# nianticlabs/mickey

Hardware: AMD Instinct MI355X
Metric: image pairs/sec (540x720) (higher is better)
Workload: dtype bf16

## Files before the change

### mickey_amd/csrc/mk_gemm_common.hpp

```cpp
#pragma once
#include "mk_common.hpp"

namespace mk {
namespace gemm {

constexpr int BK = 64;
template <typename T> constexpr int EPC = 16 / (int)sizeof(T);
template <typename T> constexpr int KT = 128 / (int)sizeof(T);

enum AMode { A_DENSE = 0, A_CONV3 = 1 };

struct GemmParams {
  const void* A;
  const void* A2;
  const void* W;
  int M, N, K, lda, ldw;
  long long strideA_g, strideA2_g, strideW_g;
  int H, Wd, C1, C2;
  int bord_out;
  unsigned pl1[2], pl2[2];
  int npass;
  float acc_scale;
  void* out_lo;
  float plane_scale;
// ... 496 lines not shown
  const int fr = lane & 15, fg = lane >> 4;
  const float* bias = HAS_BIAS ? p.bias + (long long)g * p.strideBias_g : nullptr;
  const int nw = n0 + wn * 64;
  const int mw = m0 + wm * 128;
  int img0 = 0, tok0 = 0;
  if (EPI == MK_EPI_QKV) {
    img0 = mw / p.ntok;
    tok0 = mw - img0 * p.ntok;
  }
  auto img_tok = [&](int r, int& img, int& tok) {
    if (p.ntok >= 128) {
      const int t = tok0 + r;
      const bool wrap = t >= p.ntok;
      img = img0 + (wrap ? 1 : 0);
      tok = wrap ? t - p.ntok : t;
    } else {
      const int m = mw + r;
      img = m / p.ntok;
      tok = m - img * p.ntok;
    }
  };
  f32x4 bv[4], cs[4];
#pragma unroll
  for (int ni = 0; ni < 4; ++ni) {
    const int n = nw + fg * 4 + ni * 16;
    bv[ni] = (HAS_BIAS && n < p.N) ? *(const f32x4*)(bias + n) : f32x4{0.f, 0.f, 0.f, 0.f};
    cs[ni] = (LN && n < p.N) ? *(const f32x4*)(p.ln_colsum + n) : f32x4{0.f, 0.f, 0.f, 0.f};
  }
  float2 prm[8];
#pragma unroll
  for (int mi = 0; mi < 8; ++mi) prm[mi] = LN ? lnp[wm * 128 + mi * 16 + fr] : make_float2(1.f, 0.f);
  const bool lp_out = EPI == MK_EPI_QKV || (EPI == MK_EPI_STORE && !p.out_f32 && !p.out_lo);
  if (lp_out) {
    int which = 0, head = 0;
    if (EPI == MK_EPI_QKV) {
      const int D = p.heads * 64;
      which = nw / D;
      head = (nw - which * D) >> 6;
      if (which == 2) {
#pragma unroll
        for (int mi = 0; mi < 8; ++mi) {
          const int m = mw + mi * 16 + fr;
          if (m >= p.M) continue;
          int img, tok;
          img_tok(mi * 16 + fr, img, tok);
          const long long hb = (long long)img * p.heads + head;
#pragma unroll
          for (int ni = 0; ni < 4; ++ni) {
            const f32x4 v = LN ? acc[mi][ni] * prm[mi].x + (cs[ni] * prm[mi].y + bv[ni]) : acc[mi][ni] + bv[ni];
            T* dst = (T*)p.vt + (hb * 64 + ni * 16 + fg * 4) * p.ntok_pad + vperm(tok);
#pragma unroll
            for (int e = 0; e < 4; ++e) dst[(long long)e * p.ntok_pad] = to_lp<T>(v[e]);
          }
        }
        return;
      }
    }
    const int rr = lane >> 3, c = lane & 7;
    const int n = nw + c * 8;
    const bool bord = CONV && p.bord_out;
    BorderedRow bw;
    if (bord) bw.init(mw + rr, p.H, p.Wd);
#pragma unroll
    for (int h = 0; h < 2; ++h) {
#pragma unroll
      for (int mq = 0; mq < 4; ++mq) {
        const int mi = h * 4 + mq;
        const int r = mi * 16 + fr;
        char* wrow = (mq < 2 ? wl0 : wl1) + ((mq & 1) * 16 + fr) * 128;
        const long long rrow = (CONV && p.resid_lp) ? bordered_row(min(mw + r, p.M - 1), p.H, p.Wd) : 0;
#pragma unroll
        for (int ni = 0; ni < 4; ++ni) {
          f32x4 v = acc[mi][ni];
          if (LN) v = v * prm[mi].x + (cs[ni] * prm[mi].y + bv[ni]);
          else if (HAS_BIAS) v += bv[ni];
          if (EPI == MK_EPI_QKV) {
            if (which == 0) { const float qs = p.qscale; _Pragma("unroll") for (int e = 0; e < 4; ++e) v[e] *= qs; }
          } else {
            if (CONV && p.resid_lp) {
              const int m = mw + r, n2 = nw + fg * 4 + ni * 16;
              if (m < p.M && n2 < p.N) {
                const V4 rs = *(const V4*)((const T*)p.resid_lp + (long long)g * p.strideResid_g + rrow * p.ldc + n2);
#pragma unroll
                for (int e = 0; e < 4; ++e) v[e] += (float)rs[e];
              }
            }
            if (ACT == MK_ACT_RELU) {
#pragma unroll
              for (int e = 0; e < 4; ++e) v[e] = fmaxf(v[e], 0.f);
            } else if (ACT == MK_ACT_GELU) {
              v = gelu_erf4(v);
            }
          }
          V4 o;
#pragma unroll
          for (int e = 0; e < 4; ++e) o[e] = to_lp<T>(v[e]);
          const int cc = ni * 2 + (fg >> 1);
          *(V4*)(wrow + ((cc ^ (fr & 7)) << 4) + (fg & 1) * 8) = o;
        }
      }
#pragma unroll
      for (int i8 = 0; i8 < 8; ++i8) {
        const int it = h * 8 + i8;
        const int r = it * 8 + rr;
        const int m = mw + r;
        const V8 val = *(const V8*)((i8 < 4 ? wl0 : wl1) + ((i8 & 3) * 8 + rr) * 128 + ((c ^ (rr & 7)) << 4));
        const int extra = bord ? bw.extra : 0;
        if (bord) bw.step(8, p.H, p.Wd);
        if (m >= p.M || n >= p.N) continue;
        T* dst;
        if (EPI == MK_EPI_QKV) {
          int img, tok;
          img_tok(r, img, tok);
          dst = (T*)(which == 0 ? p.q : p.k) + (((long long)img * p.heads + head) * p.ntok_pad + tok) * 64 + c * 8;
        } else {
          dst = (T*)p.out_lp + (long long)g * p.strideOut_g + ((long long)m + extra) * p.ldc + n;
        }
        if (n + 8 <= p.N) {
          *(V8*)dst = val;
        } else {
          V4 lo;
#pragma unroll
          for (int e = 0; e < 4; ++e) lo[e] = val[e];
          *(V4*)dst = lo;
        }
      }
    }
  } else {
    const int rr = lane >> 4, c = lane & 15;
    const int n = nw + c * 4;
    f32x4 gm = f32x4{0.f, 0.f, 0.f, 0.f};
    if (EPI == MK_EPI_LS_RESIDUAL && n < p.N) gm = *(const f32x4*)(p.gamma + n);
    f32x4 bvd = f32x4{0.f, 0.f, 0.f, 0.f};
    if (SPLIT && HAS_BIAS && n < p.N) bvd = *(const f32x4*)(bias + n);
    f32x4 xr[2][SPLIT ? 1 : 16];
    uint2 xh[2][SPLIT ? 16 : 1], xl[2][SPLIT ? 16 : 1];
    const unsigned lane_off = (unsigned)rr * (unsigned)p.ldxs + (unsigned)n;
    unsigned lane_off_st = lane_off;
    asm volatile("" : "+v"(lane_off_st));
    auto plane_row = [&](void* plane, int half, int it) -> T* {
      return (T*)plane + (long long)(mw + half * 64 + it * 4) * p.ldxs;
    };
    __amdgpu_buffer_rsrc_t rs_h, rs_l;
    unsigned voff_b = 0;
    if constexpr (SPLIT && EPI == MK_EPI_LS_RESIDUAL && sizeof(T) == 2) {
      rs_h = __builtin_amdgcn_make_buffer_rsrc(p.xh, 0, 0x7fffffff, 0x00020000);
      rs_l = __builtin_amdgcn_make_buffer_rsrc(p.xl, 0, 0x7fffffff, 0x00020000);
      voff_b = lane_off * 2u;
    }
    auto soff_b = [&](int half, int it) -> unsigned {
      return (unsigned)(mw + half * 64 + it * 4) * (unsigned)p.ldxs * 2u;
    };
    typedef unsigned u32x2_t __attribute__((ext_vector_type(2)));
    auto preload = [&](int half, int it0 = 0, int it1 = 16) {
      if (EPI != MK_EPI_LS_RESIDUAL) return;
#pragma unroll
      for (int it = 0; it < 16; ++it) {
        if (it < it0 || it >= it1) continue;
        const int m = mw + half * 64 + it * 4 + rr;
        const bool ok = SPLIT || (m < p.M && n < p.N);
        if constexpr (SPLIT && EPI == MK_EPI_LS_RESIDUAL && sizeof(T) == 2) {
          const u32x2_t a = __builtin_amdgcn_raw_buffer_load_b64(rs_h, voff_b, soff_b(half, it), 0);
          const u32x2_t b = __builtin_amdgcn_raw_buffer_load_b64(rs_l, voff_b, soff_b(half, it), 0);
          xh[half][it] = uint2{a[0], a[1]};
          xl[half][it] = uint2{b[0], b[1]};
        } else if (SPLIT) {
          xh[half][it] = ok ? *(const uint2*)(plane_row(p.xh, half, it) + lane_off) : uint2{0u, 0u};
          xl[half][it] = ok ? *(const uint2*)(plane_row(p.xl, half, it) + lane_off) : uint2{0u, 0u};
        } else {
          xr[half][it] = ok ? *(const f32x4*)(p.out_f32 + (long long)m * p.ldc + n) : f32x4{0.f, 0.f, 0.f, 0.f};
        }
      }
    };
    auto stageq = [&](int half, int sub) {
#pragma unroll
      for (int m2 = 0; m2 < 2; ++m2) {
        const int mi = sub * 2 + m2;
        const int r = mi * 16 + fr;
        char* wrow = (m2 == 0 ? wl0 : wl1) + fr * 256;
        const long long rrow = (CONV && p.resid_lp) ? bordered_row(min(mw + half * 64 + r, p.M - 1), p.H, p.Wd) : 0;
#pragma unroll
        for (int ni = 0; ni < 4; ++ni) {
          f32x4 v = acc[half * 4 + mi][ni];
          if (EPI == MK_EPI_STORE && p.npass > 1) {
            const float sc = p.acc_scale;
#pragma unroll
            for (int e = 0; e < 4; ++e) v[e] *= sc;
          }
          if (HAS_BIAS && !SPLIT) v += bv[ni];
          if (EPI == MK_EPI_STORE) {
            if (CONV && p.resid_lp) {
              const int m = mw + half * 64 + r, nn = nw + fg * 4 + ni * 16;
              if (m < p.M && nn < p.N) {
                const V4 rs = *(const V4*)((const T*)p.resid_lp + (long long)g * p.strideResid_g + rrow * p.ldc + nn);
#pragma unroll
                for (int e = 0; e < 4; ++e) v[e] += (float)rs[e];
              }
            }
            if (ACT == MK_ACT_RELU) {
#pragma unroll
              for (int e = 0; e < 4; ++e) v[e] = fmaxf(v[e], 0.f);
            } else if (ACT == MK_ACT_GELU) {
              v = gelu_erf4(v);
            }
          }
          const int cw = ni * 4 + fg;
          *(f32x4*)(wrow + ((cw ^ fr) << 4)) = v;
        }
      }
    };
    constexpr bool fin = FIN;
    auto emit_row = [&](long long xrow, T* dh, T* dl, f32x4 x, bool ok, unsigned soff = 0xffffffffu) {
      float ssum = 0.f, qsum = 0.f;
      if (ok) {
        const uint2 oh = pack4<T>(x);
        const uint2 ol = pack4<T>(x - unpack4<T>(oh));
        quad_stats(x, ssum, qsum);
        if constexpr (SPLIT && EPI == MK_EPI_LS_RESIDUAL && sizeof(T) == 2) {
          __builtin_amdgcn_raw_buffer_store_b64(u32x2_t{oh.x, oh.y}, rs_h, voff_b, soff, 0);
          __builtin_amdgcn_raw_buffer_store_b64(u32x2_t{ol.x, ol.y}, rs_l, voff_b, soff, 0);
        } else {
          *(uint2*)dh = oh;
          *(uint2*)dl = ol;
        }
      }
      ssum = row16_sum(ssum);
      qsum = row16_sum(qsum);
      if (ok && c == 0) ((float2*)p.stats_out)[xrow * p.nslot_out + (nw >> 6)] = make_float2(ssum, qsum);
    };
    auto drain = [&](int half, int it0 = 0, int it1 = 16) {
      const bool bordf = CONV && p.bord_out;
      BorderedRow bwf;
      if (bordf) bwf.init(mw + half * 64 + it0 * 4 + rr, p.H, p.Wd);
#pragma unroll
      for (int it = 0; it < 16; ++it) {
        if (it < it0 || it >= it1) continue;
        const int r = it * 4 + rr;
        const int m = mw + half * 64 + r;
        const int extraf = bordf ? bwf.extra : 0;
        if (bordf) bwf.step(4, p.H, p.Wd);
        f32x4 val = *(const f32x4*)(((it & 4) ? wl1 : wl0) + ((it & 3) * 4 + rr) * 256 + ((c ^ ((it & 3) * 4 + rr)) << 4));
        if (SPLIT) val += bvd;
        const bool ok = SPLIT || (m < p.M && n < p.N);
        if (!ok) continue;
        if (EPI == MK_EPI_LS_RESIDUAL) {
          f32x4 x;
          if (SPLIT) {
            x = unpack4<T>(xh[half][it]) + unpack4<T>(xl[half][it]);
          } else {
            x = xr[half][it];
          }
          x += gm * val;
          if (SPLIT) x -= ((const float*)lnp)[wm * 128 + half * 64 + r];
          if (!SPLIT || fin) {
            if (ok) *(f32x4*)(p.out_f32 + (long long)m * p.ldc + n) = x;
          } else {
            if constexpr (sizeof(T) == 2) emit_row(m, nullptr, nullptr, x, ok, soff_b(half, it));
            else emit_row(m, plane_row(p.xh, half, it) + lane_off_st, plane_row(p.xl, half, it) + lane_off_st, x, ok);
          }
        } else if (EPI == MK_EPI_PATCH) {
          const int mc = ok ? m : 0;
          const int img = mc / p.npatch, tok = mc - img * p.npatch;
          const long long xrow = (long long)img * (p.npatch + 1) + 1 + tok;
          f32x4 x = val;
          if (ok) x += *(const f32x4*)(p.pos + (long long)(1 + tok) * p.N + n);
          if (SPLIT) emit_row(xrow, (T*)p.xh + xrow * p.ldxs + n, (T*)p.xl + xrow * p.ldxs + n, x, ok);
          else if (ok) *(f32x4*)(p.out_f32 + xrow * p.ldc + n) = x;
        } else if (EPI == MK_EPI_STORE && p.out_lo) {
          const float ps = p.plane_scale;
          f16x4 oh, ol;
#pragma unroll
          for (int e = 0; e < 4; ++e) {
            const float sv = sat16(val[e] * ps, p.sat_flag);
            oh[e] = (_Float16)sv;
            ol[e] = (_Float16)(sv - (float)oh[e]);
          }
          const long long o = (long long)g * p.strideOut_g + ((long long)m + extraf) * p.ldc + n;
          *(f16x4*)((_Float16*)p.out_lp + o) = oh;
          *(f16x4*)((_Float16*)p.out_lo + o) = ol;
        } else {
          *(f32x4*)(p.out_f32 + (long long)g * p.strideOut_g + ((long long)m + extraf) * p.ldc + n) = val;
        }
      }
    };
    if (SPLIT && !FIN && EPI == MK_EPI_LS_RESIDUAL) {
      preload(0, 0, 16);
      stageq(0, 0);
      drain(0, 0, 8);
      preload(1, 0, 8);
      stageq(0, 1);
      drain(0, 8, 16);
      preload(1, 8, 16);
      stageq(1, 0);
      drain(1, 0, 8);
      stageq(1, 1);
      drain(1, 8, 16);
    } else {
      preload(0);
      stageq(0, 0);
      drain(0, 0, 8);
      stageq(0, 1);
      preload(1);
      drain(0, 8, 16);
      stageq(1, 0);
      drain(1, 0, 8);
      stageq(1, 1);
      drain(1, 8, 16);
    }
  }
}

template <typename T, int KIND, bool CONV = false, int BN = 256>
__device__ __forceinline__ void epilogue_lds(const GemmParams& p, f32x4 (&acc)[8][4], char* wl0, char* wl1, int m0, int n0, int wm,
                                             int wn, int lane, int g, const float2* lnp = nullptr) {
  if constexpr (KIND == 2 || KIND == 3) {
    const bool interior = m0 + 256 <= p.M && n0 + BN <= p.N;
    if (KIND == 3) {
      if (interior) epilogue_lds_impl<T, MK_EPI_LS_RESIDUAL, MK_ACT_NONE, true, false, true, true>(p, acc, wl0, wl1, m0, n0, wm, wn, lane, g, lnp);
      else epilogue_impl<T, 8, MK_EPI_LS_RESIDUAL, MK_ACT_NONE, true, false, true>(p, acc, m0, n0, wm, wn, lane, g);
    } else if (p.epi == MK_EPI_PATCH) {
      if (interior) epilogue_lds_impl<T, MK_EPI_PATCH, MK_ACT_NONE, true, false, true>(p, acc, wl0, wl1, m0, n0, wm, wn, lane, g);
      else epilogue_impl<T, 8, MK_EPI_PATCH, MK_ACT_NONE, true, false, true>(p, acc, m0, n0, wm, wn, lane, g);
    } else {
      if (interior) epilogue_lds_impl<T, MK_EPI_LS_RESIDUAL, MK_ACT_NONE, true, false, true, false>(p, acc, wl0, wl1, m0, n0, wm, wn, lane, g, lnp);
      else epilogue_impl<T, 8, MK_EPI_LS_RESIDUAL, MK_ACT_NONE, true, false, true>(p, acc, m0, n0, wm, wn, lane, g);
    }
  } else if constexpr (KIND == 1) {
#if defined(MK_LN_ABL) && MK_LN_ABL == 2
    constexpr bool LNE = false;
#else
    constexpr bool LNE = true;
#endif
    if (p.epi == MK_EPI_QKV) epilogue_lds_impl<T, MK_EPI_QKV, MK_ACT_NONE, true, LNE>(p, acc, wl0, wl1, m0, n0, wm, wn, lane, g, lnp);
    else if (p.act == MK_ACT_GELU) epilogue_lds_impl<T, MK_EPI_STORE, MK_ACT_GELU, true, LNE>(p, acc, wl0, wl1, m0, n0, wm, wn, lane, g, lnp);
    else epilogue_lds_impl<T, MK_EPI_STORE, MK_ACT_NONE, true, LNE>(p, acc, wl0, wl1, m0, n0, wm, wn, lane, g, lnp);
  } else {
    switch (CONV ? MK_EPI_STORE : p.epi) {
      case MK_EPI_LS_RESIDUAL: epilogue_lds_impl<T, MK_EPI_LS_RESIDUAL, MK_ACT_NONE, true>(p, acc, wl0, wl1, m0, n0, wm, wn, lane, g); break;
      case MK_EPI_QKV: epilogue_lds_impl<T, MK_EPI_QKV, MK_ACT_NONE, true>(p, acc, wl0, wl1, m0, n0, wm, wn, lane, g); break;
      case MK_EPI_PATCH: epilogue_lds_impl<T, MK_EPI_PATCH, MK_ACT_NONE, true>(p, acc, wl0, wl1, m0, n0, wm, wn, lane, g); break;
      default:
        if (!p.bias) {
          if (p.act == MK_ACT_RELU) epilogue_lds_impl<T, MK_EPI_STORE, MK_ACT_RELU, false, false, false, false, CONV>(p, acc, wl0, wl1, m0, n0, wm, wn, lane, g);
          else if (!CONV && p.act == MK_ACT_GELU) epilogue_lds_impl<T, MK_EPI_STORE, MK_ACT_GELU, false>(p, acc, wl0, wl1, m0, n0, wm, wn, lane, g);
          else epilogue_lds_impl<T, MK_EPI_STORE, MK_ACT_NONE, false, false, false, false, CONV>(p, acc, wl0, wl1, m0, n0, wm, wn, lane, g);
        } else {
          if (p.act == MK_ACT_RELU) epilogue_lds_impl<T, MK_EPI_STORE, MK_ACT_RELU, true, false, false, false, CONV>(p, acc, wl0, wl1, m0, n0, wm, wn, lane, g);
          else if (!CONV && p.act == MK_ACT_GELU) epilogue_lds_impl<T, MK_EPI_STORE, MK_ACT_GELU, true>(p, acc, wl0, wl1, m0, n0, wm, wn, lane, g);
          else epilogue_lds_impl<T, MK_EPI_STORE, MK_ACT_NONE, true, false, false, false, CONV>(p, acc, wl0, wl1, m0, n0, wm, wn, lane, g);
        }
    }
  }
}

__device__ __forceinline__ void pp_tile_coords(int id, int ntm, int ntn, int PP_GM, int& tm, int& tn) {
  if (PP_GM < 0) {
    const int ng = -PP_GM;
    const int grp = id / (ntm * ng);
    const int rem = id - grp * (ntm * ng);
    const int gn = min(ng, ntn - grp * ng);
    tm = rem / gn;
    tn = grp * ng + rem - tm * gn;
    return;
  }
  const int band = id / (PP_GM * ntn);
  const int rem = id - band * (PP_GM * ntn);
  const int gm = min(PP_GM, ntm - band * PP_GM);
  tm = band * PP_GM + rem % gm;
  tn = rem / gm;
}

int num_cus();
extern int g_pp64_persist;
int launch_pp64(const GemmParams& p, int groups, int dtype, int amode, hipStream_t st, int band_m);
int launch_f32(const GemmParams& p, int groups, int amode, hipStream_t st);

}
}
```

### mickey_amd/csrc/mk_gemm_pp64.hip

```cpp
#include <type_traits>

#include "mk_gemm_common.hpp"

namespace mk {
namespace gemm {
int g_pp64_persist = 2;
namespace {

template <typename T, int AMODE, int KIND, bool PERSIST = false, bool SP = false, bool SP2 = false>
__global__ __launch_bounds__(512, 2) void gemm_pp64_kernel(GemmParams p, int band_m) {
  static_assert(!SP2 || SP, "SP2 is a form of the split-operand kernel");
  static_assert(!PERSIST || AMODE == A_DENSE, "the persistent tile loop is built for dense operands");
  static_assert(!SP || (KIND == 0 && !PERSIST && sizeof(T) == 2), "split operands: plain epilogues, one tile per workgroup");
  constexpr int BKA = SP ? BK / 2 : BK;
  using V8 = typename Lp<T>::V8;
  constexpr int WMF = 8, BM = 256, BN = 256;
  constexpr int A_BYTES = BM * 128, STAGE_BYTES = (BM + BN) * 128;
  constexpr int LN_STAGE_OFF = 2 * STAGE_BYTES + 256 * 8;
  extern __shared__ __attribute__((aligned(16))) char smem[];

  const int tid0 = threadIdx.x;
  const int wave = __builtin_amdgcn_readfirstlane(tid0 >> 6);
  int lane = tid0 & 63, tid = tid0;
  auto refresh_lane = [&]() {
// ... 244 lines not shown

  const bool ln = KIND == 1 && p.ln_stats != nullptr;
#if defined(MK_LN_ABL) && MK_LN_ABL == 1
  const bool ln_fast = false && ln;
#define MK_LN_NO_SLOW 1
#else
  const bool ln_fast = ln && p.ln_nslot == 16;
#endif
  LnRowLoads16 lnl;
  if (ln_fast) lnl.issue(p, m0, tid);
  constexpr bool PRODUCER = AMODE == A_DENSE && (KIND == 2 || KIND == 3);
  ShiftLoad shl;
  if constexpr (PRODUCER) shl.issue(p, m0, tid, 256);
  dma_a(0);
  dma_w(0);
  if constexpr (!PERSIST) dma_a(1);
  constexpr int YOUNGER = PERSIST ? 8 : 12;
  const bool publish = ln && p.ln_shift_out != nullptr && n0 == 0;
  if (ln_fast) lnl.template finish<YOUNGER>(p, tid, (float2*)(smem + 2 * STAGE_BYTES), m0, publish);
#ifndef MK_LN_NO_SLOW
  else if (ln) ln_params_to_lds<256, 512>(p, m0, tid, (float2*)(smem + 2 * STAGE_BYTES), publish);
#endif
  if constexpr (PRODUCER) shl.template finish<YOUNGER>(tid, 256, (float*)(smem + 2 * STAGE_BYTES));
  if constexpr (!PERSIST) asm volatile("s_waitcnt vmcnt(4)" ::: "memory");
  const int bstep = PERSIST ? (int)gridDim.x : 0;
  for (;;) {
    const int nbid = bid + bstep;
    const bool has_next = PERSIST && nbid < ntiles;
    int m1 = m0, n1 = n0;
    if (PERSIST && has_next) tile_origin(nbid, m1, n1);
    if constexpr (PERSIST) {
      refresh_lane();
      derive_lane();
      set_aoff(m0);
      set_woff(n0);
      dma_a(1);
      if (bid == (int)blockIdx.x) asm volatile("s_waitcnt vmcnt(4)" ::: "memory");
    }
    bool ln_pending = false;
    auto first_stage_done = [&]() {
      if constexpr (PERSIST) {
        if (ln_pending) {
          const bool publish1 = ln && p.ln_shift_out != nullptr && n0 == 0;
          if (ln_fast) {
            LnRowDma16::finish<0>(p, wave, lane, (float2*)(smem + 2 * STAGE_BYTES), smem + LN_STAGE_OFF, m0, publish1);
            asm volatile("s_waitcnt lgkmcnt(0)" ::: "memory");
            LnRowDma16::issue<2>(p, m0, wave, lane, smem + LN_STAGE_OFF);
          }
          if constexpr (PRODUCER) shl.template finish<-1>(tid, 256, (float*)(smem + 2 * STAGE_BYTES));
        }
      }
    };
    auto second_stage_done = [&]() {
      if constexpr (PERSIST) {
        if (ln_pending && ln_fast)
          LnRowDma16::finish<2>(p, wave, lane, (float2*)(smem + 2 * STAGE_BYTES), smem + LN_STAGE_OFF, m0,
                                ln && p.ln_shift_out != nullptr && n0 == 0);
      }
    };
    ln_pending = PERSIST && bid != (int)blockIdx.x;
    int kt0 = 0;
    if (wm == 0) {
      if constexpr (PERSIST) {
        stage0(0, Yes{}, Yes{}, 1, 2, Yes{});
        first_stage_done();
        stage0(1, Yes{}, Yes{}, 2, 3, No{});
        second_stage_done();
        kt0 = 2;
      }
      for (int kt = kt0; kt < nk - 2; ++kt) stage0(kt, Yes{}, Yes{}, kt + 1, kt + 2, No{});
      if constexpr (PERSIST) {
        set_aoff(m1);
        stage0(nk - 2, Yes{}, Yes{}, nk - 1, 0, No{});
        set_woff(n1);
        stage0(nk - 1, Yes{}, No{}, 0, 0, No{});
      } else {
        stage0(nk - 2, Yes{}, No{}, nk - 1, 0, No{});
        stage0(nk - 1, No{}, No{}, 0, 0, No{});
      }
      bar();
    } else {
      bar();
      if constexpr (PERSIST) {
        stage1(0, Yes{}, Yes{}, 1, 2, Yes{});
        first_stage_done();
        stage1(1, Yes{}, Yes{}, 2, 3, No{});
        second_stage_done();
        kt0 = 2;
      }
      for (int kt = kt0; kt < nk - 2; ++kt) stage1(kt, Yes{}, Yes{}, kt + 1, kt + 2, No{});
      if constexpr (PERSIST) {
        set_aoff(m1);
        stage1(nk - 2, Yes{}, Yes{}, nk - 1, 0, No{});
        set_woff(n1);
        stage1(nk - 1, Yes{}, No{}, 0, 0, No{});
      } else {
        stage1(nk - 2, Yes{}, No{}, nk - 1, 0, No{});
        stage1(nk - 1, No{}, No{}, 0, 0, No{});
      }
    }
    char* wl0 = smem + STAGE_BYTES + wave * 4096;
    refresh_lane();
    epilogue_lds<T, KIND, AMODE == A_CONV3>(p, acc, wl0, wl0 + A_BYTES, m0, n0, wm, wn, lane, g, (const float2*)(smem + 2 * STAGE_BYTES));
    if (!(PERSIST && has_next)) break;
    bid = nbid;
    m0 = m1;
    n0 = n1;
    asm volatile("" : "+s"(m0), "+s"(n0));
    refresh_lane();
    if (ln_fast) LnRowDma16::issue<0>(p, m0, wave, lane, smem + LN_STAGE_OFF);
    if constexpr (PRODUCER) shl.issue(p, m0, tid, 256);
  }
}

template <typename T, int AMODE, int KIND, bool PERSIST, bool SP = false, bool SP2 = false>
int launch_k2(const GemmParams& p, int groups, hipStream_t st, int band_m, int grid) {
  constexpr int LDS = 2 * 512 * 128 + 256 * 8 + (PERSIST && KIND == 1 ? 16384 : 0);
  static bool attr_done = false;
  if (!attr_done) {
    hipError_t e = hipFuncSetAttribute((const void*)gemm_pp64_kernel<T, AMODE, KIND, PERSIST, SP, SP2>, hipFuncAttributeMaxDynamicSharedMemorySize, LDS);
    if (e != hipSuccess) {
      mk_set_error("gemm: cannot reserve %d B of LDS: %s", LDS, hipGetErrorString(e));
      return MK_ERR_LAUNCH;
    }
    attr_done = true;
  }
  hipLaunchKernelGGL((gemm_pp64_kernel<T, AMODE, KIND, PERSIST, SP, SP2>), dim3(grid, groups, 1), dim3(512), LDS, st, p, band_m);
  MK_CHECK_LAUNCH();
  return MK_OK;
}

template <typename T, int AMODE, int KIND>
int launch_k(const GemmParams& p, int groups, hipStream_t st, int band_m) {
  const int ntm = (p.M + 255) / 256, ntn = (p.N + 255) / 256;
  if (band_m == 0) band_m = (AMODE == A_DENSE && ntn <= 4) ? -4 : 8;
  if constexpr (KIND == 0 && sizeof(T) == 2 && std::is_same<T, _Float16>::value) {
    if (p.npass == 2) {
      if constexpr (AMODE == A_CONV3) return launch_k2<T, AMODE, 0, false, true, true>(p, groups, st, band_m, ntm * ntn);
    }
    if (p.npass > 1) return launch_k2<T, AMODE, 0, false, true>(p, groups, st, band_m, ntm * ntn);
  }
  if constexpr (AMODE == A_DENSE && KIND != 0) {
    const int nk = p.K / BK, grid = num_cus() & ~7;
    const bool ok = groups == 1 && p.npass <= 1 && (nk & 1) == 0 && nk >= 4 && grid >= 8 && ntm * ntn > grid &&
                    !(KIND == 1 && p.ln_stats && p.ln_nslot != 16);
    if (g_pp64_persist != 1 && ok && !(g_pp64_persist == 2 && KIND == 1)) return launch_k2<T, AMODE, KIND, true>(p, groups, st, band_m, grid);
  }
  return launch_k2<T, AMODE, KIND, false>(p, groups, st, band_m, ntm * ntn);
}

template <typename T>
int launch_dense(const GemmParams& p, int groups, hipStream_t st, int band_m) {
  if (p.xh && p.epi == MK_EPI_LS_RESIDUAL && p.out_f32) return launch_k<T, A_DENSE, 3>(p, groups, st, band_m);
  if (p.xh) return launch_k<T, A_DENSE, 2>(p, groups, st, band_m);
  if (p.ln_stats) return launch_k<T, A_DENSE, 1>(p, groups, st, band_m);
  return launch_k<T, A_DENSE, 0>(p, groups, st, band_m);
}

}

int launch_pp64(const GemmParams& p, int groups, int dtype, int amode, hipStream_t st, int band_m) {
  if (amode == A_DENSE) return dtype == MK_BF16 ? launch_dense<__bf16>(p, groups, st, band_m) : launch_dense<_Float16>(p, groups, st, band_m);
  return dtype == MK_BF16 ? launch_k<__bf16, A_CONV3, 0>(p, groups, st, band_m) : launch_k<_Float16, A_CONV3, 0>(p, groups, st, band_m);
}

}
}
```

### mickey_amd/csrc/mk_norm.hip

```cpp
#include "mk_common.hpp"
#include "mk_gemm_common.hpp"

#include <stdarg.h>
#include <stdio.h>

namespace {
using namespace mk;

__device__ __forceinline__ void store_planes(void* hi, void* lo, long long o, const f32x4& y, float scale, int* sat_flag) {
  f16x4 oh, ol;
#pragma unroll
  for (int e = 0; e < 4; ++e) {
    const float sv = sat16(y[e] * scale, sat_flag);
    oh[e] = (_Float16)sv;
    ol[e] = (_Float16)(sv - (float)oh[e]);
  }
  *(f16x4*)((_Float16*)hi + o) = oh;
  if (lo) *(f16x4*)((_Float16*)lo + o) = ol;
}

constexpr int LN_MAXV = 8;

constexpr int LN_RPW = 4;

// ... 138 lines not shown
    if (r < rows_out && cok) {
      const long long rin = (long long)(r / rpo) * rows_per_img + skip + (r % rpo);
      v[t] = __builtin_nontemporal_load((const f32x4*)(x + rin * ldx + c));
    }
  }
#pragma unroll
  for (int t = 0; t < LNN_TRIPS; ++t) {
    const int r = r0 + 2 * t + half;
    const bool ok = r < rows_out && cok;
    float mean, rstd;
    f32x4 d;
    ln_narrow_stats(v[t], cok, D, eps, mean, rstd, d);
    if (!ok) continue;
    const long long wo = wgroup_rows > 0 ? (long long)(r / wgroup_rows) * D : 0;
    const f32x4 ww = *(const f32x4*)(w + wo + c), bb = *(const f32x4*)(b + wo + c);
    f32x4 y;
#pragma unroll
    for (int e = 0; e < 4; ++e) y[e] = ln_scale(d[e], rstd, ww[e], bb[e]);
    if (resid) {
      float* rp = resid + (long long)r * ldr + c;
      y += *(const f32x4*)rp;
      *(f32x4*)rp = y;
    }
    if (out) {
      long long ro = r;
      if (bord_h > 0) {
        const int gb = r / bord_m, m = r - gb * bord_m;
        ro = gb * bordered_rows(bord_m / (bord_h * bord_w), bord_h, bord_w) + bordered_row(m, bord_h, bord_w);
      }
      if (out_is_f32 == 2) {
        store_planes(out, out_lo, ro * ldo + c, y, plane_scale, sat_flag);
      } else if (out_is_f32) {
        *(f32x4*)((float*)out + ro * ldo + c) = y;
      } else {
        typename Lp<T>::V4 o;
#pragma unroll
        for (int e = 0; e < 4; ++e) o[e] = (T)y[e];
        *(typename Lp<T>::V4*)((T*)out + ro * ldo + c) = o;
      }
    }
  }
}

constexpr int NCHW_TP = 64;
constexpr int NCHW_CC = 128;
constexpr int NCHW_LD = NCHW_TP + 1;
template <int MAXV, bool NARROW>
__global__ __launch_bounds__(256) void layernorm_nchw_kernel(const float* __restrict__ x, int ldx, const float* __restrict__ w,
                                                             const float* __restrict__ b, float eps, float* __restrict__ out,
                                                             int npix, int D, int rows_per_img, int skip, int tiles, int round_fp16) {
  __shared__ float tile[NCHW_CC * NCHW_LD];
  __shared__ float s_mean[NCHW_TP], s_rstd[NCHW_TP];
  const int tid = threadIdx.x, lane = tid & 63, wave = tid >> 6;
  const int img = blockIdx.x / tiles, p0 = (blockIdx.x - img * tiles) * NCHW_TP;
  const int np = min(NCHW_TP, npix - p0);
  const float* xt = x + ((long long)img * rows_per_img + skip + p0) * ldx;
  if constexpr (NARROW) {
    constexpr int TRIPS = NCHW_TP / 8;
    const int half = lane >> 5, c = (lane & 31) * 4;
    const bool cok = c < D;
#pragma unroll 1
    for (int t0 = 0; t0 < TRIPS; t0 += LNN_TRIPS) {
      f32x4 v[LNN_TRIPS];
#pragma unroll
      for (int t = 0; t < LNN_TRIPS; ++t) {
        const int p = (wave * TRIPS + t0 + t) * 2 + half;
        v[t] = f32x4{0.f, 0.f, 0.f, 0.f};
        if (p < np && cok) v[t] = *(const f32x4*)(xt + (long long)p * ldx + c);
      }
#pragma unroll
      for (int t = 0; t < LNN_TRIPS; ++t) {
        const int p = (wave * TRIPS + t0 + t) * 2 + half;
        float mean, rstd;
        f32x4 d;
        ln_narrow_stats(v[t], cok, D, eps, mean, rstd, d);
        if ((lane & 31) == 0 && p < np) {
          s_mean[p] = mean;
          s_rstd[p] = rstd;
        }
      }
    }
  } else {
    constexpr int RPW = NCHW_TP / 4;
    f32x4 v[2][MAXV];
    auto load_row = [&](int p, f32x4 (&dst)[MAXV]) {
      const float* xr = xt + (long long)p * ldx;
#pragma unroll
      for (int i = 0; i < MAXV; ++i) {
        const int c = (i * 64 + lane) * 4;
        if (c < D) dst[i] = *(const f32x4*)(xr + c);
      }
    };
    auto step = [&](int p, f32x4 (&cur)[MAXV], f32x4 (&nxt)[MAXV]) {
      if (p >= np) return;
      if (p + 4 < np) load_row(p + 4, nxt);
      float mean, rstd;
      ln_row_stats<MAXV>(cur, lane, D, eps, mean, rstd);
      if (lane == 0) {
        s_mean[p] = mean;
        s_rstd[p] = rstd;
      }
    };
    if (wave < np) load_row(wave, v[0]);
#pragma unroll 1
    for (int rr = 0; rr < RPW; rr += 2) {
      step(rr * 4 + wave, v[0], v[1]);
      step(rr * 4 + 4 + wave, v[1], v[0]);
    }
  }
  __syncthreads();
#pragma unroll 1
  for (int c0 = 0; c0 < D; c0 += NCHW_CC) {
#pragma unroll 1
    for (int hb = 0; hb < NCHW_CC / 64; ++hb) {
      const int cl = hb * 64 + (tid & 15) * 4, c = c0 + cl;
      if (c < D) {
        const f32x4 ww = *(const f32x4*)(w + c), bb = *(const f32x4*)(b + c);
        f32x4 xv[4];
#pragma unroll
        for (int j = 0; j < 4; ++j) {
          const int p = j * 16 + (tid >> 4);
          if (p < np) xv[j] = __builtin_nontemporal_load((const f32x4*)(xt + (long long)p * ldx + c));
        }
#pragma unroll
        for (int j = 0; j < 4; ++j) {
          const int p = j * 16 + (tid >> 4);
          if (p < np) {
            const float mean = s_mean[p], rstd = s_rstd[p];
#pragma unroll
            for (int e = 0; e < 4; ++e) {
              float y = ln_norm(xv[j][e], mean, rstd, ww[e], bb[e]);
              if (round_fp16) {
                asm volatile("" : "+v"(y));
                y = (float)(_Float16)y;
              }
              tile[(cl + e) * NCHW_LD + p] = y;
            }
          }
        }
      }
    }
    __syncthreads();
#pragma unroll 8
    for (int it = 0; it < NCHW_CC * NCHW_TP / 256; ++it) {
      const int idx = it * 256 + tid;
      const int cl = idx >> 6, p = idx & (NCHW_TP - 1);
      const int c = c0 + cl;
      if (p < np && c < D) out[((long long)img * D + c) * npix + p0 + p] = tile[cl * NCHW_LD + p];
    }
    __syncthreads();
  }
}

template <typename T>
__global__ __launch_bounds__(256) void im2col14_kernel(const float* __restrict__ img, long long stride_img,
                                                       long long stride_ch, int stride_row, int nimg, int gh, int gw,
                                                       T* __restrict__ out, int ldo) {
  const int cols4 = ldo >> 2;
  const long long total = (long long)nimg * gh * gw * cols4;
  for (long long i = blockIdx.x * (long long)blockDim.x + threadIdx.x; i < total; i += (long long)gridDim.x * blockDim.x) {
    const int c4 = (int)(i % cols4);
    const long long m = i / cols4;
    const int pc = (int)(m % gw);
    const int pr = (int)((m / gw) % gh);
    const int im = (int)(m / ((long long)gw * gh));
    typename Lp<T>::V4 o;
#pragma unroll
    for (int e = 0; e < 4; ++e) {
      const int k = c4 * 4 + e;
      float v = 0.f;
      if (k < 588) {
        const int ch = k / 196, rem = k - ch * 196, dy = rem / 14, dx = rem - dy * 14;
        v = img[im * stride_img + ch * stride_ch + (long long)(pr * 14 + dy) * stride_row + pc * 14 + dx];
      }
      o[e] = (T)v;
    }
    *(typename Lp<T>::V4*)(out + m * ldo + c4 * 4) = o;
  }
}

__global__ void cls_kernel(const float* __restrict__ cls, const float* __restrict__ pos, float* __restrict__ x, int nimg,
                           int ntok, int D) {
  const int i = blockIdx.x * blockDim.x + threadIdx.x;
  if (i >= nimg * D) return;
  const int im = i / D, c = i - im * D;
  x[(long long)im * ntok * D + c] = cls[c] + pos[c];
}

template <typename T>
__global__ __launch_bounds__(64) void cls_ln_kernel(const float* __restrict__ cls, const float* __restrict__ pos, T* __restrict__ xh,
                                                    T* __restrict__ xl, float* __restrict__ stats, int ntok, int D) {
  const int im = blockIdx.x, lane = threadIdx.x;
  const long long row = (long long)im * ntok;
  for (int c0 = 0; c0 < D; c0 += 64) {
    const float v = cls[c0 + lane] + pos[c0 + lane];
    const T h = (T)v;
    xh[row * D + c0 + lane] = h;
    xl[row * D + c0 + lane] = (T)(v - (float)h);
    const float s = mk::wave_sum(v), q = mk::wave_sum(v * v);
    if (lane == 0) ((float2*)stats)[row * (D / 64) + (c0 >> 6)] = make_float2(s, q);
  }
}

template <typename T>
__global__ __launch_bounds__(256) void recentre_kernel(T* __restrict__ xh, T* __restrict__ xl, float* __restrict__ stats,
                                                       long long rows, int D) {
  using V4 = typename mk::Lp<T>::V4;
  const int lane = threadIdx.x & 63;
  const long long row = (long long)blockIdx.x * 4 + (threadIdx.x >> 6);
  if (row >= rows) return;
  const int nslot = D >> 6;
  T* ph = xh + row * D;
  T* pl = xl + row * D;
  const int quad = lane & 15, sub = lane >> 4;
  float sum = 0.f;
  for (int s0 = 0; s0 < nslot; s0 += 4) {
    const int slot = s0 + sub;
    if (slot < nslot) {
      const V4 h = *(const V4*)(ph + slot * 64 + quad * 4), l = *(const V4*)(pl + slot * 64 + quad * 4);
#pragma unroll
      for (int e = 0; e < 4; ++e) sum += (float)h[e] + (float)l[e];
    }
  }
  const float mean = mk::wave_sum(sum) / (float)D;
  for (int s0 = 0; s0 < nslot; s0 += 4) {
    const int slot = s0 + sub;
    const bool ok = slot < nslot;
    f32x4 x = f32x4{0.f, 0.f, 0.f, 0.f};
    if (ok) {
      const V4 h = *(const V4*)(ph + slot * 64 + quad * 4), l = *(const V4*)(pl + slot * 64 + quad * 4);
      V4 oh, ol;
#pragma unroll
      for (int e = 0; e < 4; ++e) {
        x[e] = ((float)h[e] + (float)l[e]) - mean;
        oh[e] = (T)x[e];
        ol[e] = (T)(x[e] - (float)oh[e]);
      }
      *(V4*)(ph + slot * 64 + quad * 4) = oh;
      *(V4*)(pl + slot * 64 + quad * 4) = ol;
    }
    float s, q;
    mk::gemm::quad_stats(x, s, q);
    s = mk::gemm::row16_sum(s);
    q = mk::gemm::row16_sum(q);
    if (ok && quad == 0) ((float2*)stats)[row * nslot + slot] = make_float2(s, q);
  }
}

}

static thread_local char g_err[512] = "";
void mk_set_error(const char* fmt, ...) {
  va_list ap;
  va_start(ap, fmt);
  vsnprintf(g_err, sizeof(g_err), fmt, ap);
  va_end(ap);
}

extern "C" {

int mk_version(void) { return 100; }

const char* mk_last_error(void) { return g_err; }

static int layernorm_launch(const float* x, int ldx, const float* w, const float* b, float eps, void* out, int ldo, int out_is_f32,
                            float* resid, int ldr, int rows_out, int D, int rows_per_img, int skip, int wgroup_rows, int bord_h,
                            int bord_w, int bord_m, int dtype, void* out_lo, float plane_scale, int* sat_flag, mk_stream_t stream) {
  MK_CHECK_ARG(x && w && b && (out || resid), "mk_layernorm: null pointer");
  MK_CHECK_ARG(bord_h == 0 || (bord_h > 0 && bord_w > 0 && bord_m > 0 && bord_m % (bord_h * bord_w) == 0 && rows_out % bord_m == 0),
               "mk_layernorm: bordered output needs rows_out = k * bord_m, bord_m = nimg * bord_h * bord_w");
  MK_CHECK_ARG(D > 0 && D % 4 == 0 && D <= LN_MAXV * 256, "mk_layernorm: D=%d must be a multiple of 4 and <= %d", D,
               LN_MAXV * 256);
  MK_CHECK_ARG(rows_out > 0 && rows_per_img > skip && skip >= 0 && ldx % 4 == 0 && ldo % 4 == 0 && ldr % 4 == 0,
               "mk_layernorm: bad geometry");
  MK_CHECK_ARG(ldx >= D && (!out || ldo >= D) && (!resid || ldr >= D),
               "mk_layernorm: leading dimensions (ldx=%d ldo=%d ldr=%d) must be >= D=%d", ldx, ldo, ldr, D);
  if (D <= 128) {
    dim3 gridn((rows_out + 8 * LNN_TRIPS - 1) / (8 * LNN_TRIPS));
#define MK_LNN(T_)                                                                                                         \
  hipLaunchKernelGGL((layernorm_narrow_kernel<T_>), gridn, dim3(256), 0, (hipStream_t)stream, x, ldx, w, b, eps, out, ldo, \
                     out_is_f32, resid, ldr, rows_out, D, rows_per_img, skip, wgroup_rows, bord_h, bord_w, bord_m, out_lo, plane_scale, sat_flag)
    if (dtype == MK_BF16) MK_LNN(__bf16);
    else if (dtype == MK_F16) MK_LNN(_Float16);
    else MK_LNN(float);
#undef MK_LNN
    MK_CHECK_LAUNCH();
    return MK_OK;
  }
  dim3 grid((rows_out + 4 * LN_RPW - 1) / (4 * LN_RPW));
#define MK_LN(T_, V_)                                                                                                  \
  hipLaunchKernelGGL((layernorm_kernel<T_, V_>), grid, dim3(256), 0, (hipStream_t)stream, x, ldx, w, b, eps, out, ldo, \
                     out_is_f32, resid, ldr, rows_out, D, rows_per_img, skip, wgroup_rows, bord_h, bord_w, bord_m, out_lo, plane_scale, sat_flag)
  if (dtype == MK_BF16) {
    if (D <= 1024) MK_LN(__bf16, 4); else MK_LN(__bf16, LN_MAXV);
  } else if (dtype == MK_F16) {
    if (D <= 1024) MK_LN(_Float16, 4); else MK_LN(_Float16, LN_MAXV);
  } else {
    if (D <= 1024) MK_LN(float, 4); else MK_LN(float, LN_MAXV);
  }
#undef MK_LN
  MK_CHECK_LAUNCH();
  return MK_OK;
}

int mk_layernorm(const float* x, int ldx, const float* w, const float* b, float eps, void* out, int ldo, int out_is_f32,
                 float* resid, int ldr, int rows_out, int D, int rows_per_img, int skip, int wgroup_rows, int bord_h,
                 int bord_w, int bord_m, int dtype, mk_stream_t stream) {
  return layernorm_launch(x, ldx, w, b, eps, out, ldo, out_is_f32 ? 1 : 0, resid, ldr, rows_out, D, rows_per_img, skip, wgroup_rows,
                          bord_h, bord_w, bord_m, dtype, nullptr, 1.0f, nullptr, stream);
}

int mk_layernorm_planes(const float* x, int ldx, const float* w, const float* b, float eps, void* out_hi, void* out_lo, int ldo,
                        float plane_scale, float* resid, int ldr, int rows_out, int D, int rows_per_img, int skip, int wgroup_rows,
                        int bord_h, int bord_w, int bord_m, int* sat_flag, mk_stream_t stream) {
  MK_CHECK_ARG(out_hi, "mk_layernorm_planes: null plane pointer");
  return layernorm_launch(x, ldx, w, b, eps, out_hi, ldo, 2, resid, ldr, rows_out, D, rows_per_img, skip, wgroup_rows, bord_h, bord_w,
                          bord_m, MK_F32, out_lo, plane_scale, sat_flag, stream);
}

int mk_layernorm_nchw(const float* x, int ldx, const float* w, const float* b, float eps, float* out, int nimg, int npix, int D,
                      int rows_per_img, int skip, int round_fp16, mk_stream_t stream) {
  MK_CHECK_ARG(x && w && b && out, "mk_layernorm_nchw: null pointer");
  MK_CHECK_ARG(D > 0 && D % 4 == 0 && D <= LN_MAXV * 256, "mk_layernorm_nchw: D=%d must be a multiple of 4 and <= %d", D,
               LN_MAXV * 256);
  MK_CHECK_ARG(nimg > 0 && npix > 0 && skip >= 0 && rows_per_img >= skip + npix && ldx >= D && ldx % 4 == 0,
               "mk_layernorm_nchw: bad geometry (nimg=%d npix=%d rows_per_img=%d skip=%d ldx=%d)", nimg, npix, rows_per_img, skip, ldx);
  const int tiles = (npix + NCHW_TP - 1) / NCHW_TP;
  MK_CHECK_ARG((long long)nimg * tiles <= 0x7fffffffLL, "mk_layernorm_nchw: too many tiles");
  const dim3 grid((unsigned)(nimg * tiles));
#define MK_LNT(V_, N_)                                                                                                      \
  hipLaunchKernelGGL((layernorm_nchw_kernel<V_, N_>), grid, dim3(256), 0, (hipStream_t)stream, x, ldx, w, b, eps, out, npix, D, \
                     rows_per_img, skip, tiles, round_fp16 ? 1 : 0)
  if (D <= 128) MK_LNT(4, true);
  else if (D <= 1024) MK_LNT(4, false);
  else MK_LNT(LN_MAXV, false);
#undef MK_LNT
  MK_CHECK_LAUNCH();
  return MK_OK;
}

int mk_im2col_patch14(const float* img, long long stride_img, long long stride_ch, int stride_row, int nimg, int gh,
                      int gw, void* out, int ldo, int dtype, mk_stream_t stream) {
  MK_CHECK_ARG(img && out && nimg > 0 && gh > 0 && gw > 0, "mk_im2col_patch14: bad args");
  MK_CHECK_ARG(ldo >= 588 && ldo % 8 == 0, "mk_im2col_patch14: ldo=%d must be >= 588 and a multiple of 8", ldo);
  const long long total = (long long)nimg * gh * gw * (ldo / 4);
  int blocks = (int)((total + 255) / 256);
  if (blocks > 16384) blocks = 16384;
  if (dtype == MK_BF16)
    hipLaunchKernelGGL(im2col14_kernel<__bf16>, dim3(blocks), dim3(256), 0, (hipStream_t)stream, img, stride_img, stride_ch,
                       stride_row, nimg, gh, gw, (__bf16*)out, ldo);
  else if (dtype == MK_F16)
    hipLaunchKernelGGL(im2col14_kernel<_Float16>, dim3(blocks), dim3(256), 0, (hipStream_t)stream, img, stride_img,
                       stride_ch, stride_row, nimg, gh, gw, (_Float16*)out, ldo);
  else
    hipLaunchKernelGGL(im2col14_kernel<float>, dim3(blocks), dim3(256), 0, (hipStream_t)stream, img, stride_img,
                       stride_ch, stride_row, nimg, gh, gw, (float*)out, ldo);
  MK_CHECK_LAUNCH();
  return MK_OK;
}

int mk_cls_token(const float* cls, const float* pos, float* x, int nimg, int ntok, int D, mk_stream_t stream) {
  MK_CHECK_ARG(cls && pos && x && nimg > 0 && ntok > 0 && D > 0, "mk_cls_token: bad args");
  hipLaunchKernelGGL(cls_kernel, dim3((nimg * D + 255) / 256), dim3(256), 0, (hipStream_t)stream, cls, pos, x, nimg, ntok, D);
  MK_CHECK_LAUNCH();
  return MK_OK;
}

int mk_cls_token_ln(const float* cls, const float* pos, void* xh, void* xl, float* stats, int nimg, int ntok, int D, int dtype,
                    mk_stream_t stream) {
  MK_CHECK_ARG(cls && pos && xh && xl && stats && nimg > 0 && ntok > 0 && D > 0 && D % 64 == 0, "mk_cls_token_ln: bad args");
  MK_CHECK_ARG(dtype == MK_BF16 || dtype == MK_F16, "mk_cls_token_ln: 16-bit dtypes only");
  if (dtype == MK_BF16)
    hipLaunchKernelGGL((cls_ln_kernel<__bf16>), dim3(nimg), dim3(64), 0, (hipStream_t)stream, cls, pos, (__bf16*)xh, (__bf16*)xl, stats, ntok, D);
  else
    hipLaunchKernelGGL((cls_ln_kernel<_Float16>), dim3(nimg), dim3(64), 0, (hipStream_t)stream, cls, pos, (_Float16*)xh, (_Float16*)xl, stats, ntok, D);
  MK_CHECK_LAUNCH();
  return MK_OK;
}

int mk_recentre_split(void* xh, void* xl, float* stats, long long rows, int D, int dtype, mk_stream_t stream) {
  MK_CHECK_ARG(xh && xl && stats && rows > 0 && D > 0 && D % 64 == 0, "mk_recentre_split: bad args");
  MK_CHECK_ARG(dtype == MK_BF16 || dtype == MK_F16, "mk_recentre_split: 16-bit dtypes only");
  const dim3 grid((unsigned)((rows + 3) / 4));
  if (dtype == MK_BF16)
    hipLaunchKernelGGL((recentre_kernel<__bf16>), grid, dim3(256), 0, (hipStream_t)stream, (__bf16*)xh, (__bf16*)xl, stats, rows, D);
  else
    hipLaunchKernelGGL((recentre_kernel<_Float16>), grid, dim3(256), 0, (hipStream_t)stream, (_Float16*)xh, (_Float16*)xl, stats, rows, D);
  MK_CHECK_LAUNCH();
  return MK_OK;
}

}
```

Baseline: 279.7.

## Specialize patch-embed epilogue with buffer ops and stage im2col through LDS

Adds a dedicated GEMM kernel kind for the patch-embedding epilogue. It preloads position embeddings with buffer loads interleaved into the LDS drain schedule and walks token indices incrementally instead of dividing per row, and it writes the split hi/lo planes and row stats with buffer stores. Separately, it rewrites the im2col kernel so each block loads a chunk of a patch row into shared memory with vectorized coalesced reads, then writes 16-byte output vectors. Both changes target the patch-embed front end, which is a small part of the total work, at the cost of more complex index arithmetic.

```diff
diff --git a/mickey_amd/csrc/mk_gemm_common.hpp b/mickey_amd/csrc/mk_gemm_common.hpp
--- a/mickey_amd/csrc/mk_gemm_common.hpp
+++ b/mickey_amd/csrc/mk_gemm_common.hpp
@@ -672,6 +672,61 @@
       return (unsigned)(mw + half * 64 + it * 4) * (unsigned)p.ldxs * 2u;
     };
     typedef unsigned u32x2_t __attribute__((ext_vector_type(2)));
+    constexpr bool PBUF = SPLIT && EPI == MK_EPI_PATCH && sizeof(T) == 2;
+    struct PatchWalk {
+      int tok;
+      unsigned dx;
+      __device__ __forceinline__ void step(int np, int q4, int r4) {
+        tok += r4;
+        asm volatile("" : "+s"(tok));
+        const int w = tok >= np ? 1 : 0;
+        tok -= np & -w;
+        dx += 4u + (unsigned)q4 + (unsigned)w;
+      }
+    };
+    __amdgpu_buffer_rsrc_t rs_s, rs_p;
+    PatchWalk pw_ld = {0, 0u}, pw_st = {0, 0u};
+    int np = 1, q4 = 0, r4 = 0, pthr = 0, ptk0 = 0, ptk1 = 0;
+    unsigned pv0 = 0, pv1 = 0, ps0 = 0, ps1 = 0, pn4 = 0, rowb = 0, srowb = 0, posb = 0;
+    f32x4 pe[PBUF ? 2 : 1][PBUF ? 16 : 1];
+    if constexpr (PBUF) {
+      np = p.npatch;
+      const int img0 = __builtin_amdgcn_readfirstlane(mw / np);
+      const int tok0 = __builtin_amdgcn_readfirstlane(mw - img0 * np);
+      const long long xrow0 = (long long)mw + img0 + 1;
+      rowb = (unsigned)p.ldxs * 2u;
+      srowb = (unsigned)p.nslot_out * 8u;
+      posb = (unsigned)p.N * 4u;
+      rs_h = __builtin_amdgcn_make_buffer_rsrc((char*)p.xh + xrow0 * rowb, 0, 0x7fffffff, 0x00020000);
+      rs_l = __builtin_amdgcn_make_buffer_rsrc((char*)p.xl + xrow0 * rowb, 0, 0x7fffffff, 0x00020000);
+      rs_s = __builtin_amdgcn_make_buffer_rsrc((char*)p.stats_out + (xrow0 * p.nslot_out + (nw >> 6)) * 8, 0, 0x7fffffff, 0x00020000);
+      rs_p = __builtin_amdgcn_make_buffer_rsrc((void*)p.pos, 0, 0x7fffffff, 0x00020000);
+      pw_ld.tok = pw_st.tok = tok0;
+      q4 = __builtin_amdgcn_readfirstlane((np <= 4 ? 1 : 0) + (2 * np <= 4 ? 1 : 0) + (3 * np <= 4 ? 1 : 0) + (np == 1 ? 1 : 0));
+      r4 = 4 - q4 * np;
+      const int qr = (rr >= np ? 1 : 0) + (rr >= 2 * np ? 1 : 0) + (rr >= 3 * np ? 1 : 0);
+      const int rrm = rr - qr * np;
+      pthr = np - rrm;
+      ptk0 = rrm + 1;
+      ptk1 = rrm + 1 - np;
+      pn4 = (unsigned)n * 4u;
+      pv0 = (unsigned)(rr + qr) * rowb + (unsigned)n * 2u;
+      pv1 = pv0 + rowb;
+      ps0 = (unsigned)(rr + qr) * srowb;
+      ps1 = ps0 + srowb;
+    }
+    auto pos_preload = [&](int half, int it0, int it1) {
+      if constexpr (PBUF) {
+#pragma unroll
+        for (int it = 0; it < 16; ++it) {
+          if (it < it0 || it >= it1) continue;
+          const int t = pw_ld.tok + (pw_ld.tok >= pthr ? ptk1 : ptk0);
+          const u32x4 v = __builtin_amdgcn_raw_buffer_load_b128(rs_p, __umul24((unsigned)t, posb) + pn4, 0, 0);
+          pe[half][it] = __builtin_bit_cast(f32x4, v);
+          pw_ld.step(np, q4, r4);
+        }
+      }
+    };
     auto preload = [&](int half, int it0 = 0, int it1 = 16) {
       if (EPI != MK_EPI_LS_RESIDUAL) return;
 #pragma unroll
@@ -778,6 +833,24 @@
             if constexpr (sizeof(T) == 2) emit_row(m, nullptr, nullptr, x, ok, soff_b(half, it));
             else emit_row(m, plane_row(p.xh, half, it) + lane_off_st, plane_row(p.xl, half, it) + lane_off_st, x, ok);
           }
+        } else if (PBUF) {
+          if constexpr (PBUF) {
+            const bool wl = pw_st.tok >= pthr;
+            const f32x4 x = val + pe[half][it];
+            const uint2 oh = pack4<T>(x);
+            const uint2 ol = pack4<T>(x - unpack4<T>(oh));
+            float ssum, qsum;
+            quad_stats(x, ssum, qsum);
+            const unsigned so = pw_st.dx * rowb, vo = wl ? pv1 : pv0;
+            __builtin_amdgcn_raw_buffer_store_b64(u32x2_t{oh.x, oh.y}, rs_h, vo, so, 0);
+            __builtin_amdgcn_raw_buffer_store_b64(u32x2_t{ol.x, ol.y}, rs_l, vo, so, 0);
+            ssum = row16_sum(ssum);
+            qsum = row16_sum(qsum);
+            if (c == 0)
+              __builtin_amdgcn_raw_buffer_store_b64(u32x2_t{__builtin_bit_cast(unsigned, ssum), __builtin_bit_cast(unsigned, qsum)}, rs_s,
+                                                    wl ? ps1 : ps0, pw_st.dx * srowb, 0);
+            pw_st.step(np, q4, r4);
+          }
         } else if (EPI == MK_EPI_PATCH) {
           const int mc = ok ? m : 0;
           const int img = mc / p.npatch, tok = mc - img * p.npatch;
@@ -812,6 +885,19 @@
       drain(0, 8, 16);
       preload(1, 8, 16);
       stageq(1, 0);
+      drain(1, 0, 8);
+      stageq(1, 1);
+      drain(1, 8, 16);
+    } else if (PBUF) {
+      pos_preload(0, 0, 8);
+      stageq(0, 0);
+      pos_preload(0, 8, 16);
+      drain(0, 0, 8);
+      stageq(0, 1);
+      pos_preload(1, 0, 8);
+      drain(0, 8, 16);
+      stageq(1, 0);
+      pos_preload(1, 8, 16);
       drain(1, 0, 8);
       stageq(1, 1);
       drain(1, 8, 16);
@@ -833,14 +919,15 @@
 template <typename T, int KIND, bool CONV = false, int BN = 256>
 __device__ __forceinline__ void epilogue_lds(const GemmParams& p, f32x4 (&acc)[8][4], char* wl0, char* wl1, int m0, int n0, int wm,
                                              int wn, int lane, int g, const float2* lnp = nullptr) {
-  if constexpr (KIND == 2 || KIND == 3) {
+  if constexpr (KIND == 4) {
+    const bool interior = m0 + 256 <= p.M && n0 + BN <= p.N;
+    if (interior) epilogue_lds_impl<T, MK_EPI_PATCH, MK_ACT_NONE, true, false, true>(p, acc, wl0, wl1, m0, n0, wm, wn, lane, g);
+    else epilogue_impl<T, 8, MK_EPI_PATCH, MK_ACT_NONE, true, false, true>(p, acc, m0, n0, wm, wn, lane, g);
+  } else if constexpr (KIND == 2 || KIND == 3) {
     const bool interior = m0 + 256 <= p.M && n0 + BN <= p.N;
     if (KIND == 3) {
       if (interior) epilogue_lds_impl<T, MK_EPI_LS_RESIDUAL, MK_ACT_NONE, true, false, true, true>(p, acc, wl0, wl1, m0, n0, wm, wn, lane, g, lnp);
       else epilogue_impl<T, 8, MK_EPI_LS_RESIDUAL, MK_ACT_NONE, true, false, true>(p, acc, m0, n0, wm, wn, lane, g);
-    } else if (p.epi == MK_EPI_PATCH) {
-      if (interior) epilogue_lds_impl<T, MK_EPI_PATCH, MK_ACT_NONE, true, false, true>(p, acc, wl0, wl1, m0, n0, wm, wn, lane, g);
-      else epilogue_impl<T, 8, MK_EPI_PATCH, MK_ACT_NONE, true, false, true>(p, acc, m0, n0, wm, wn, lane, g);
     } else {
       if (interior) epilogue_lds_impl<T, MK_EPI_LS_RESIDUAL, MK_ACT_NONE, true, false, true, false>(p, acc, wl0, wl1, m0, n0, wm, wn, lane, g, lnp);
       else epilogue_impl<T, 8, MK_EPI_LS_RESIDUAL, MK_ACT_NONE, true, false, true>(p, acc, m0, n0, wm, wn, lane, g);
diff --git a/mickey_amd/csrc/mk_gemm_pp64.hip b/mickey_amd/csrc/mk_gemm_pp64.hip
--- a/mickey_amd/csrc/mk_gemm_pp64.hip
+++ b/mickey_amd/csrc/mk_gemm_pp64.hip
@@ -420,6 +420,7 @@
 template <typename T>
 int launch_dense(const GemmParams& p, int groups, hipStream_t st, int band_m) {
   if (p.xh && p.epi == MK_EPI_LS_RESIDUAL && p.out_f32) return launch_k<T, A_DENSE, 3>(p, groups, st, band_m);
+  if (p.xh && p.epi == MK_EPI_PATCH) return launch_k<T, A_DENSE, 4>(p, groups, st, band_m);
   if (p.xh) return launch_k<T, A_DENSE, 2>(p, groups, st, band_m);
   if (p.ln_stats) return launch_k<T, A_DENSE, 1>(p, groups, st, band_m);
   return launch_k<T, A_DENSE, 0>(p, groups, st, band_m);
diff --git a/mickey_amd/csrc/mk_norm.hip b/mickey_amd/csrc/mk_norm.hip
--- a/mickey_amd/csrc/mk_norm.hip
+++ b/mickey_amd/csrc/mk_norm.hip
@@ -314,31 +314,67 @@
   }
 }
 
-template <typename T>
+constexpr int IM2_P = 16, IM2_LD = 656;
+template <typename T, int VL>
 __global__ __launch_bounds__(256) void im2col14_kernel(const float* __restrict__ img, long long stride_img,
                                                        long long stride_ch, int stride_row, int nimg, int gh, int gw,
-                                                       T* __restrict__ out, int ldo) {
-  const int cols4 = ldo >> 2;
-  const long long total = (long long)nimg * gh * gw * cols4;
-  for (long long i = blockIdx.x * (long long)blockDim.x + threadIdx.x; i < total; i += (long long)gridDim.x * blockDim.x) {
-    const int c4 = (int)(i % cols4);
-    const long long m = i / cols4;
-    const int pc = (int)(m % gw);
-    const int pr = (int)((m / gw) % gh);
-    const int im = (int)(m / ((long long)gw * gh));
-    typename Lp<T>::V4 o;
-#pragma unroll
-    for (int e = 0; e < 4; ++e) {
-      const int k = c4 * 4 + e;
-      float v = 0.f;
-      if (k < 588) {
-        const int ch = k / 196, rem = k - ch * 196, dy = rem / 14, dx = rem - dy * 14;
-        v = img[im * stride_img + ch * stride_ch + (long long)(pr * 14 + dy) * stride_row + pc * 14 + dx];
-      }
-      o[e] = (T)v;
-    }
-    *(typename Lp<T>::V4*)(out + m * ldo + c4 * 4) = o;
-  }
+                                                       T* __restrict__ out, int ldo, int pchunk, int nchunk) {
+  constexpr int E = 16 / (int)sizeof(T);
+  typedef T TV __attribute__((ext_vector_type(VL)));
+  typedef float FV __attribute__((ext_vector_type(VL)));
+  typedef T T16 __attribute__((ext_vector_type(E)));
+  __shared__ __attribute__((aligned(16))) T tile[IM2_P * IM2_LD];
+  const int tid = threadIdx.x;
+  int b = blockIdx.x;
+  const int ck = b % nchunk;
+  b /= nchunk;
+  const int pr = b % gh, im = b / gh;
+  const int pc0 = ck * pchunk;
+  const int np = min(pchunk, gw - pc0);
+  const long long m0 = ((long long)im * gh + pr) * gw + pc0;
+  if (E == 8 && tid < np) *(uint2*)(tile + tid * IM2_LD + 588) = uint2{0u, 0u};
+  constexpr int RUN = IM2_P * 14 / VL;
+  constexpr int SLOT = VL == 2 ? 128 : 256, RPP = 256 / SLOT, NPASS = 42 / RPP;
+  const int j = tid & (SLOT - 1);
+  const int pj = j / (14 / VL), dxj = (j - pj * (14 / VL)) * VL;
+  const bool act = j < np * (14 / VL);
+  const float* src = img + im * stride_img + (long long)pr * 14 * stride_row + pc0 * 14 + j * VL;
+  T* dst = tile + pj * IM2_LD + dxj;
+  FV v[NPASS] = {};
+#pragma unroll
+  for (int ps = 0; ps < NPASS; ++ps) {
+    const int r = ps * RPP + (RPP == 2 ? tid >> 7 : 0);
+    const int ch = r / 14, dy = r - ch * 14;
+    if (act) v[ps] = *(const FV*)(src + ch * stride_ch + (long long)dy * stride_row);
+  }
+#pragma unroll
+  for (int ps = 0; ps < NPASS; ++ps) {
+    const int r = ps * RPP + (RPP == 2 ? tid >> 7 : 0);
+    TV o;
+#pragma unroll
+    for (int e = 0; e < VL; ++e) o[e] = (T)v[ps][e];
+    if (act) *(TV*)(dst + r * 14) = o;
+  }
+  __syncthreads();
+  const int nch = ldo / E, total = np * nch;
+  const int qs = 256 / nch, rs = 256 - qs * nch;
+  int row = tid / nch, pcs = tid - row * nch;
+  T* o16 = out + m0 * ldo;
+  for (int i = tid; i < total; i += 256) {
+    T16 val;
+    if (pcs * E < 588) {
+      val = *(const T16*)(tile + row * IM2_LD + pcs * E);
+    } else {
+#pragma unroll
+      for (int e = 0; e < E; ++e) val[e] = (T)0.f;
+    }
+    *(T16*)(o16 + (long long)i * E) = val;
+    pcs += rs;
+    const bool w = pcs >= nch;
+    pcs -= w ? nch : 0;
+    row += qs + (w ? 1 : 0);
+  }
+  static_assert(RUN <= SLOT && 42 % RPP == 0, "a run fits its slot");
 }
 
 __global__ void cls_kernel(const float* __restrict__ cls, const float* __restrict__ pos, float* __restrict__ x, int nimg,
@@ -505,18 +541,19 @@
                       int gw, void* out, int ldo, int dtype, mk_stream_t stream) {
   MK_CHECK_ARG(img && out && nimg > 0 && gh > 0 && gw > 0, "mk_im2col_patch14: bad args");
   MK_CHECK_ARG(ldo >= 588 && ldo % 8 == 0, "mk_im2col_patch14: ldo=%d must be >= 588 and a multiple of 8", ldo);
-  const long long total = (long long)nimg * gh * gw * (ldo / 4);
-  int blocks = (int)((total + 255) / 256);
-  if (blocks > 16384) blocks = 16384;
-  if (dtype == MK_BF16)
-    hipLaunchKernelGGL(im2col14_kernel<__bf16>, dim3(blocks), dim3(256), 0, (hipStream_t)stream, img, stride_img, stride_ch,
-                       stride_row, nimg, gh, gw, (__bf16*)out, ldo);
-  else if (dtype == MK_F16)
-    hipLaunchKernelGGL(im2col14_kernel<_Float16>, dim3(blocks), dim3(256), 0, (hipStream_t)stream, img, stride_img,
-                       stride_ch, stride_row, nimg, gh, gw, (_Float16*)out, ldo);
-  else
-    hipLaunchKernelGGL(im2col14_kernel<float>, dim3(blocks), dim3(256), 0, (hipStream_t)stream, img, stride_img,
-                       stride_ch, stride_row, nimg, gh, gw, (float*)out, ldo);
+  MK_CHECK_ARG(dtype == MK_BF16 || dtype == MK_F16 || dtype == MK_F32, "mk_im2col_patch14: bad dtype %d", dtype);
+  MK_CHECK_ARG((uintptr_t)out % 16 == 0, "mk_im2col_patch14: out must be 16-byte aligned");
+  const int nchunk = (gw + IM2_P - 1) / IM2_P, pchunk = (gw + nchunk - 1) / nchunk;
+  const long long blocks = (long long)nimg * gh * nchunk;
+  MK_CHECK_ARG(blocks < (1ll << 31), "mk_im2col_patch14: too many patch rows");
+  const bool v2 = (uintptr_t)img % 8 == 0 && stride_img % 2 == 0 && stride_ch % 2 == 0 && stride_row % 2 == 0;
+#define MK_IM2(T_, VL_)                                                                                                      \
+  hipLaunchKernelGGL((im2col14_kernel<T_, VL_>), dim3((unsigned)blocks), dim3(256), 0, (hipStream_t)stream, img, stride_img, \
+                     stride_ch, stride_row, nimg, gh, gw, (T_*)out, ldo, pchunk, nchunk)
+  if (dtype == MK_BF16) { if (v2) MK_IM2(__bf16, 2); else MK_IM2(__bf16, 1); }
+  else if (dtype == MK_F16) { if (v2) MK_IM2(_Float16, 2); else MK_IM2(_Float16, 1); }
+  else { if (v2) MK_IM2(float, 2); else MK_IM2(float, 1); }
+#undef MK_IM2
   MK_CHECK_LAUNCH();
   return MK_OK;
 }
```

After: 279.5, median of 2. Within noise of the previous version (-0.1%).
